# jmhb0/view_neti

Hardware: AMD Instinct MI355X
Metric: TI train steps/sec (SD-1.5 512^2 bs=4 per GPU) (higher is better)
Workload: dtype f16; 1 GPU; learnable_mode 0, sd15 shapes, 512x512 fp16, bs=4/GPU, grad_accum 1, full train step (VAE+16xCLIP+UNet fwd/bwd+AdamW); global_batch=4, parallelism=dp1, rccl_ranks=1, hipgraph=True

## Files before the change

### include/vneti.h

```cpp
#ifndef VNETI_H
#define VNETI_H
#include <stddef.h>
#include <stdint.h>

#ifdef __cplusplus
extern "C" {
#endif

#define VNETI_ABI_VERSION 1

int vneti_version(void);
int vneti_precision(void);
int vneti_last_error(char* buf, size_t n);

typedef struct vneti_gemm_desc {
  const void* A;
  const void* B;
  void* C;
  long long lda, ldb, ldc;
  int M, N, K;
  int batch;
  long long strideA, strideB, strideC;
  const float* bias;
  const void* rowadd;
// ... 65 lines not shown
int vneti_groupnorm_bwd(const void* dy, long long lddy, const void* x, long long ldx,
                        const float* gamma, const float* beta, const float* mean,
                        const float* rstd, void* dx, long long lddx, const void* dx_accum,
                        long long ldacc, float* ws, int Bn, int HW, int C, int G, int silu,
                        void* stream);

int vneti_layernorm_fwd(const void* x, int x_is_f32, long long ldx, void* y, long long ldy,
                        const float* gamma, const float* beta, float* mean, float* rstd, int rows,
                        int C, float eps, void* stream);
int vneti_layernorm_bwd(const void* dy, int dy_is_f32, long long lddy, const void* x,
                        int x_is_f32, long long ldx, const float* gamma, const float* mean,
                        const float* rstd, void* dx, int dx_is_f32, long long lddx,
                        const void* dx_accum, long long ldacc, void* dx_f16_copy, long long ldcopy,
                        int rows, int C, void* stream);

int vneti_attn_fwd(const void* Q, long long ldq, const void* K, long long ldk, const void* V,
                   long long ldv, void* O, long long ldo, float* lse, int Bn, int H, int Nq,
                   int Nk, int D, float scale, int causal, void* stream);
int vneti_attn_bwd_delta(const void* dO, long long lddo, const void* O, long long ldo,
                         float* delta, int Bn, int H, int Nq, int D, void* stream);
int vneti_attn_bwd_dq(const void* Q, long long ldq, const void* K, long long ldk, const void* V,
                      long long ldv, const void* dO, long long lddo, const float* lse, float* delta,
                      const void* O, long long ldo, void* dQ, long long lddq, int Bn, int H, int Nq,
                      int Nk, int D, float scale, int causal, void* stream);
int vneti_attn_bwd_dkv(const void* Q, long long ldq, const void* K, long long ldk, const void* V,
                       long long ldv, const void* dO, long long lddo, const float* lse,
                       const float* delta, void* dK, long long lddk, void* dV, long long lddv,
                       int Bn, int H, int Nq, int Nk, int D, float scale, int causal, float* ws,
                       long long ws_floats, void* stream);
int vneti_attn_bwd_small(const void* Q, long long ldq, const void* K, long long ldk, const void* V, long long ldv,
                         const void* dO, long long lddo, const void* O, long long ldo, const float* lse, void* dQ,
                         long long lddq, void* dK, long long lddk, void* dV, long long lddv, int Bn, int H, int N, int D,
                         float scale, int causal, void* stream);
int vneti_softmax_rows_f16(void* x, long long ld, int rows, int cols, void* stream);

int vneti_add_f16(const void* a, long long lda, const void* b, long long ldb, void* out,
                  long long ldo, int rows, int cols, void* stream);
int vneti_geglu_fwd(const void* p, long long ldp, void* out, long long ldo, int rows, int C4,
                    void* stream);
int vneti_geglu_bwd(const void* dy, long long lddy, const void* p, long long ldp, void* dp,
                    long long lddp, int rows, int C4, void* stream);
int vneti_act_fwd_f16(const void* x, void* y, long long n, int act, void* stream);
int vneti_act_bwd_f16(const void* dy, const void* x, void* dx, long long n, int act, void* stream);
int vneti_timestep_embedding(const void* t, void* out, int Bn, int dim, void* stream);
int vneti_sum2x2_f16(const void* in, long long ldi, void* out, long long ldo, int Bn, int H, int W,
                     int C, void* stream);
int vneti_rng_fill_normal(void* out_f32, long long n, const void* state, unsigned stream_id,
                          void* stream);
int vneti_rng_fill_randint(void* out_i64, int n, int high, const void* state, unsigned stream_id,
                           void* stream);
int vneti_rng_advance(void* state, void* stream);
int vneti_nested_dropout_mask(float* mask, int nl, int Bn, int hidden, float prob, const void* state,
                              unsigned stream_id, void* stream);
int vneti_sample_add_noise(const void* moments, long long ldm, const float* eps,
                           const float* noise, const void* timesteps_i64,
                           const float* alphas_cumprod, float scaling, int v_prediction,
                           float* latents, float* noisy, float* target, int Bn, int Lc, int HW,
                           void* stream);
int vneti_latent_sample(const void* moments, long long ldm, const float* eps, float scaling, float* latents, int Bn,
                        int Lc, int HW, void* stream);
int vneti_add_noise(const float* latents, const float* noise, const void* timesteps_i64, const float* alphas_cumprod,
                    int v_prediction, float* noisy, float* target, int Bn, int Lc, int HW, void* stream);
int vneti_cfg_sampler_step(const void* pred, long long ldp, float* x, float* m_prev, float* x_in, int Bn,
                           int Lc, int HW, float guidance, float alpha_t, float sigma_t, float cx,
                           float c0, float c1, int v_prediction, void* stream);
int vneti_cfg_sampler_step_table(const void* pred, long long ldp, float* x, float* m_prev, float* x_in,
// ... 135 lines not shown
```

### view_neti_amd/csrc/attention.hip

```cpp
#include "common.h"
#include "../../include/vneti.h"

namespace {

constexpr float LOG2E = 1.4426950408889634f;
constexpr int TROW64 = 144;
constexpr int TROW32 = 80;
constexpr int DKV_QH(int D) { return D <= 64 ? 2 : 1; }

template <int D>
struct Cfg {
  static constexpr int KS = (D + 15) / 16;
  static constexpr int DPAD = KS * 16;
  static constexpr int DB = (D + 31) / 32;
  static constexpr int DCH = D / 8;
  static constexpr int ROW = DPAD * 2 + 16;
};

struct AttnArgs {
  const half_t *Q, *K, *V, *dO;
  half_t *O, *dQ, *dK, *dV;
  float* lse;
  const float* lse_in;
  const float* delta;
  float* delta_out;
  const half_t* O_in;
  long long ldq, ldk, ldv, ldo, lddo, lddq, lddk, lddv;
  int Bn, H, Nq, Nk, D;
  float scale;
  int causal;
  int qsplit;
  float* ws;
};

__device__ __forceinline__ float fast_exp2(float x) { return __builtin_amdgcn_exp2f(x); }
typedef float f32x2 __attribute__((ext_vector_type(2)));
__device__ __forceinline__ f32x2 pk_fma(f32x2 a, f32x2 b, f32x2 c) { return __builtin_elementwise_fma(a, b, c); }

constexpr float RESCALE_THR_LOG2 = 8.0f * 1.4426950408889634f;

__device__ __forceinline__ void zero_lds(char* smem, int bytes) {
  u32x4 z = {0u, 0u, 0u, 0u};
  for (int i = threadIdx.x * 16; i < bytes; i += 256 * 16) *reinterpret_cast<u32x4*>(smem + i) = z;
}

__device__ __forceinline__ half8 cvt8(const f32x16& v, int j) {
  half8 h;
#pragma unroll
  for (int e = 0; e < 8; ++e) h[e] = (half_t)v[8 * j + e];
  return h;
}

typedef short vn_short4 __attribute__((__vector_size__(4 * sizeof(short))));
__device__ __forceinline__ half8 load_tr(const char* tile, int row_bytes, int d0, int n0, int lane) {
  const int i = lane & 15;
  const char* p = tile + (n0 + (i >> 2)) * row_bytes + (d0 + 16 * ((lane >> 4) & 1) + 4 * (i & 3)) * 2;
  typedef __attribute__((address_space(3))) vn_short4* lds_ptr;
  vn_short4 lo = __builtin_amdgcn_ds_read_tr16_b64_v4i16((lds_ptr)(p));
  vn_short4 hi = __builtin_amdgcn_ds_read_tr16_b64_v4i16((lds_ptr)(p + 8 * row_bytes));
  half4 l4 = __builtin_bit_cast(half4, lo), h4 = __builtin_bit_cast(half4, hi);
  half8 r = {l4[0], l4[1], l4[2], l4[3], h4[0], h4[1], h4[2], h4[3]};
  return r;
}

template <int D, int QW>
// ... 797 lines not shown
      for (int j = 0; j < 2; ++j) {
        half8 pf = cvt8(s, j);
        half8 dsf = cvt8(dp, j);
#pragma unroll
        for (int db = 0; db < C::DB; ++db) {
          half8 dot = load_tr(dOs, C::ROW, db * 32, hq * 32 + 16 * j + 4 * h2, lane);
          half8 qtf = load_tr(Qs, C::ROW, db * 32, hq * 32 + 16 * j + 4 * h2, lane);
          dv[db] = VN_MFMA_32x32x16(dot, pf, dv[db], 0, 0, 0);
          dk[db] = VN_MFMA_32x32x16(qtf, dsf, dk[db], 0, 0, 0);
        }
      }
    }
    if (rok) {
      half_t* krow = a.dK + ((long long)b * N + row) * a.lddk + h * D;
      half_t* vrow = a.dV + ((long long)b * N + row) * a.lddv + h * D;
#pragma unroll
      for (int db = 0; db < C::DB; ++db)
#pragma unroll
        for (int qd = 0; qd < 4; ++qd) {
          const int d = db * 32 + 8 * qd + 4 * h2;
          if (d < D) {
            half4 k4 = {(half_t)(dk[db][4 * qd] * a.scale), (half_t)(dk[db][4 * qd + 1] * a.scale),
                        (half_t)(dk[db][4 * qd + 2] * a.scale), (half_t)(dk[db][4 * qd + 3] * a.scale)};
            half4 v4 = {(half_t)dv[db][4 * qd], (half_t)dv[db][4 * qd + 1], (half_t)dv[db][4 * qd + 2],
                        (half_t)dv[db][4 * qd + 3]};
            *reinterpret_cast<half4*>(krow + d) = k4;
            *reinterpret_cast<half4*>(vrow + d) = v4;
          }
        }
    }
  }
}

__global__ __launch_bounds__(256) void attn_dkv_reduce_kernel(AttnArgs a) {
  const int Cc = a.H * a.D;
  const long long rows = (long long)a.Bn * a.Nk;
  const long long plane = rows * Cc;
  const unsigned gid = blockIdx.x * 256u + threadIdx.x;
  if (gid >= (unsigned)(plane / 4)) return;
  const unsigned e32 = gid * 4u;
  const unsigned row32 = e32 / (unsigned)Cc;
  const int c = (int)(e32 - row32 * (unsigned)Cc);
  const long long e = e32, row = row32;
  f32x4 k = {0.f, 0.f, 0.f, 0.f}, v = {0.f, 0.f, 0.f, 0.f};
  for (int s = 0; s < a.qsplit; ++s) {
    k += *reinterpret_cast<const f32x4*>(a.ws + ((long long)s * 2) * plane + e);
    v += *reinterpret_cast<const f32x4*>(a.ws + ((long long)s * 2 + 1) * plane + e);
  }
  half4 k4 = {(half_t)(k[0] * a.scale), (half_t)(k[1] * a.scale), (half_t)(k[2] * a.scale), (half_t)(k[3] * a.scale)};
  half4 v4 = {(half_t)v[0], (half_t)v[1], (half_t)v[2], (half_t)v[3]};
  *reinterpret_cast<half4*>(a.dK + row * a.lddk + c) = k4;
  *reinterpret_cast<half4*>(a.dV + row * a.lddv + c) = v4;
}

int check_common(int Bn, int H, int Nq, int Nk, int D) {
  if (Bn <= 0 || H <= 0 || Nq <= 0 || Nk <= 0) return -1;
  if (!(D == 40 || D == 64 || D == 80 || D == 160)) return -2;
  return 0;
}

#define DISPATCH_D(KERNEL, grid, st, args)                                                   \
  switch (args.D) {                                                                          \
    case 40: hipLaunchKernelGGL((KERNEL<40>), grid, dim3(256), 0, st, args); break;          \
    case 64: hipLaunchKernelGGL((KERNEL<64>), grid, dim3(256), 0, st, args); break;          \
    case 80: hipLaunchKernelGGL((KERNEL<80>), grid, dim3(256), 0, st, args); break;          \
    default: hipLaunchKernelGGL((KERNEL<160>), grid, dim3(256), 0, st, args); break;         \
  }

#define DISPATCH_D1(KERNEL, grid, st, args)                                                     \
  switch (args.D) {                                                                             \
    case 40: hipLaunchKernelGGL((KERNEL<40, 1>), grid, dim3(256), 0, st, args); break;          \
    case 64: hipLaunchKernelGGL((KERNEL<64, 1>), grid, dim3(256), 0, st, args); break;          \
    case 80: hipLaunchKernelGGL((KERNEL<80, 1>), grid, dim3(256), 0, st, args); break;          \
    default: hipLaunchKernelGGL((KERNEL<160, 1>), grid, dim3(256), 0, st, args); break;         \
  }

}

extern "C" int vneti_attn_fwd(const void* Q, long long ldq, const void* K, long long ldk, const void* V,
                              long long ldv, void* O, long long ldo, float* lse, int Bn, int H, int Nq, int Nk,
                              int D, float scale, int causal, void* stream) {
  int rc = check_common(Bn, H, Nq, Nk, D);
  VN_REQUIRE(rc == 0, "attn_fwd: unsupported shape B=%d H=%d Nq=%d Nk=%d D=%d", Bn, H, Nq, Nk, D);
  VN_REQUIRE(Q && K && V && O, "attn_fwd: null pointer");
  VN_REQUIRE(ldq % 8 == 0 && ldk % 8 == 0 && ldv % 8 == 0 && ldo % 4 == 0, "attn_fwd: bad strides");
  AttnArgs a;
  memset(&a, 0, sizeof(a));
  a.Q = (const half_t*)Q;
  a.K = (const half_t*)K;
  a.V = (const half_t*)V;
  a.O = (half_t*)O;
  a.lse = lse;
  a.ldq = ldq;
  a.ldk = ldk;
// ... 65 lines not shown
extern "C" int vneti_attn_bwd_dkv(const void* Q, long long ldq, const void* K, long long ldk, const void* V,
                                  long long ldv, const void* dO, long long lddo, const float* lse, const float* delta,
                                  void* dK, long long lddk, void* dV, long long lddv, int Bn, int H, int Nq,
                                  int Nk, int D, float scale, int causal, float* ws, long long ws_floats,
                                  void* stream) {
  int rc = check_common(Bn, H, Nq, Nk, D);
  VN_REQUIRE(rc == 0, "attn_bwd_dkv: unsupported shape B=%d H=%d Nq=%d Nk=%d D=%d", Bn, H, Nq, Nk, D);
  VN_REQUIRE(Q && K && V && dO && lse && delta && dK && dV, "attn_bwd_dkv: null pointer");
  VN_REQUIRE(ldq % 8 == 0 && ldk % 8 == 0 && ldv % 8 == 0 && lddo % 8 == 0 && lddk % 4 == 0 && lddv % 4 == 0,
             "attn_bwd_dkv: bad strides");
  AttnArgs a;
  memset(&a, 0, sizeof(a));
  a.Q = (const half_t*)Q;
  a.K = (const half_t*)K;
  a.V = (const half_t*)V;
  a.dO = (const half_t*)dO;
  a.dK = (half_t*)dK;
  a.dV = (half_t*)dV;
  a.lse_in = lse;
  a.delta = delta;
  a.ldq = ldq;
  a.ldk = ldk;
  a.ldv = ldv;
  a.lddo = lddo;
  a.lddk = lddk;
  a.lddv = lddv;
  a.Bn = Bn;
  a.H = H;
  a.Nq = Nq;
  a.Nk = Nk;
  a.D = D;
  a.scale = scale;
  a.causal = causal;
  const int nkb = cdiv(Nk, 128), nqt = cdiv(Nq, 32 * DKV_QH(D));
  long long blocks = (long long)nkb * H * Bn;
  int qsplit = 1;
  if (ws && !causal && blocks <= 256 && nqt >= 8) {
    qsplit = (int)(512 / blocks);
    if (qsplit > nqt / 4) qsplit = nqt / 4;
    if (qsplit > 32) qsplit = 32;
    const long long plane = (long long)Bn * Nk * H * D;
    while (qsplit > 1 && (2LL * qsplit * plane > ws_floats || 8LL * qsplit * plane >= (1LL << 32) - 64)) --qsplit;
    if (qsplit < 2) qsplit = 1;
  }
  a.qsplit = qsplit;
  a.ws = ws;
  dim3 grid(nkb * qsplit, H, Bn);
  hipStream_t st = (hipStream_t)stream;
  DISPATCH_D(attn_dkv_kernel, grid, st, a);
  if (qsplit > 1) {
    long long n4 = (long long)Bn * Nk * H * D / 4;
    VN_REQUIRE(n4 * 4 < 0x7fffffffLL, "attn_bwd_dkv: q-split reduce indexes with 32 bits");
    hipLaunchKernelGGL(attn_dkv_reduce_kernel, dim3((unsigned)cdivl(n4, 256)), dim3(256), 0, st, a);
  }
  return vneti_check_launch("attn_bwd_dkv");
}

extern "C" int vneti_attn_bwd_small(const void* Q, long long ldq, const void* K, long long ldk, const void* V, long long ldv,
                                    const void* dO, long long lddo, const void* O, long long ldo, const float* lse, void* dQ,
                                    long long lddq, void* dK, long long lddk, void* dV, long long lddv, int Bn, int H, int N,
                                    int D, float scale, int causal, void* stream) {
  VN_REQUIRE(Q && K && V && dO && O && lse && dQ && dK && dV, "attn_bwd_small: null pointer");
  VN_REQUIRE(Bn > 0 && H > 0 && N > 0, "attn_bwd_small: bad shape B=%d H=%d N=%d", Bn, H, N);
  if (N > 96 || D != 64) return VNETI_EUNSUP;
  VN_REQUIRE(ldq % 8 == 0 && ldk % 8 == 0 && ldv % 8 == 0 && lddo % 8 == 0 && ldo % 8 == 0 && lddq % 4 == 0 && lddk % 4 == 0 &&
                 lddv % 4 == 0, "attn_bwd_small: bad strides");
  AttnArgs a;
  memset(&a, 0, sizeof(a));
  a.Q = (const half_t*)Q;
  a.K = (const half_t*)K;
  a.V = (const half_t*)V;
  a.dO = (const half_t*)dO;
  a.O_in = (const half_t*)O;
  a.lse_in = lse;
  a.dQ = (half_t*)dQ;
  a.dK = (half_t*)dK;
  a.dV = (half_t*)dV;
  a.ldq = ldq;
  a.ldk = ldk;
  a.ldv = ldv;
  a.lddo = lddo;
  a.ldo = ldo;
  a.lddq = lddq;
  a.lddk = lddk;
  a.lddv = lddv;
  a.Bn = Bn;
  a.H = H;
  a.Nq = N;
// ... 8 lines not shown
```

### view_neti_amd/engine/schedule.py

```python
from __future__ import annotations

from functools import partial
from typing import Dict, List

import torch

from .. import lib, ops, packing


class T:

    __slots__ = ("v", "g", "gw", "rows", "cols", "children", "need_grad", "producer")

    def __init__(self, v, g=None, need_grad=True):
        self.v = v
        self.g = g
        self.gw = False
        self.rows, self.cols = v.shape
        self.children: List["T"] = []
        self.need_grad = need_grad
        self.producer = None


def rup(x, m):
# ... 135 lines not shown
        conv = f.keywords.get("conv")
        B_cm = packing._chunk_major(f.args[1], f.args[1].shape[0], conv["Ci"]) if _chunk_major_ok(conv) else None
        best, best_t = (0, 0, 0), float("inf")
        for h, sk, ko in gemm_variants(key, conv, f.keywords.get("geglu"), candidates):
            kw = dict(f.keywords)
            kw["tile_hint"], kw["split_k"] = h, sk
            args = f.args
            if ko:
                kw["conv"] = dict(conv, korder=1)
                args = (f.args[0], B_cm) + tuple(f.args[2:])
            t = _time_call(partial(ops.gemm, *args, **kw), args[0], *how)
            if t < best_t:
                best, best_t = (h, sk, ko), t
        return best, B_cm

    def _pin(self, f, pick, B_cm=None):
        pick = tuple(pick) + (0,) * (3 - len(pick))
        conv = f.keywords.get("conv")
        kw = dict(f.keywords)
        kw["tile_hint"], kw["split_k"] = pick[0], pick[1]
        args = f.args
        if pick[2] and _chunk_major_ok(conv):
            if B_cm is None:
                B_cm = packing._chunk_major(f.args[1], f.args[1].shape[0], conv["Ci"])
            kw["conv"] = dict(conv, korder=1)
            self.bytes += B_cm.numel() * B_cm.element_size()
            args = (f.args[0], B_cm) + tuple(f.args[2:])
        return partial(ops.gemm, *args, **kw)

    def bind_workspace(self):
        for lst in (self.fwd_pre, self.fwd, self.bwd):
            for idx, f in enumerate(lst):
                fn = getattr(f, "func", None)
                if fn is ops.gemm or fn is ops.attn_bwd_dkv:
                    lst[idx] = self._rebound(f, fn, dict(f.keywords, workspace=self.ws))

    @staticmethod
    def _rebound(f, fn, kw):
        return partial(fn, *f.args, **kw)

    GN_SLOTS = 8

    def _produced(self, t: T):
        t.producer = len(self.fwd) - 1
        return t

    GN2_MAX = 512

    def _gn2_slice(self):
        if not hasattr(self, "_gn2_arena"):
            self._gn2_arena = self._buf((self.GN2_MAX, self.B, self.GN_SLOTS, self.groups, 4), torch.int64, zero=True)
            self._gn2_used = 0
        assert self._gn2_used < self.GN2_MAX
        self._gn2_used += 1
        return self._gn2_arena[self._gn2_used - 1]

    def fuse_gn_stats(self, fuse: bool = True):
        n = self._fuse_gn_stats() if fuse else 0
        if getattr(self, "_gn2_used", 0):
            self.fwd.insert(0, self._gn2_arena[:self._gn2_used].zero_)
        return n

    def _fuse_gn_stats(self):
        import os
        if os.environ.get("VNETI_NO_GN_FUSE"):
            return 0
        S, G, B = self.GN_SLOTS, self.groups, self.B
# ... 263 lines not shown
```

### view_neti_amd/engine/unet.py

```python
from __future__ import annotations

from functools import partial
from typing import Dict

import torch

from .. import ops, packing
from .. import sd_config as sc
from .schedule import Schedule, T, rup as _rup


class UNetEngine(Schedule):
    def __init__(self, cfg: sc.UNetConfig, weights: Dict[str, torch.Tensor], batch: int, height: int, width: int,
                 ctx_len: int = 77, device: str = "cuda", need_backward: bool = True, autotune: bool = True,
                 fuse_gn: bool = True):
        super().__init__(batch, cfg.norm_num_groups, cfg.norm_eps, device, need_backward)
        self.cfg = cfg
        self.H, self.W = height, width
        self.L = ctx_len
        self.nl = cfg.n_cross_layers
        B, L, Dc = batch, ctx_len, cfg.cross_attention_dim
        self.x_in = self._buf((B, cfg.in_channels, height, width), torch.float32)
        self.timesteps = torch.zeros(B, dtype=torch.int64, device=device)
        self.ctx_k = self._buf((self.nl, B * L, Dc))
# ... 154 lines not shown
            run["wkd"][slot].copy_(w[t + "attn2.to_k.weight"].t())
            run["wvd"][slot].copy_(w[t + "attn2.to_v.weight"].t())
            r["w_outd"] = tr(w[name + "proj_out.weight"].reshape(Cc, Cc))
            r["wff2d"], r["wff1d"] = tr(w[t + "ff.net.2.weight"]), tr(wff1_il)
            r["wo2d"] = tr(w[t + "attn2.to_out.0.weight"])
            if need_dx:
                r["wq2d"] = tr(w[t + "attn2.to_q.weight"])
                r["wo1d"] = tr(w[t + "attn1.to_out.0.weight"])
                r["wqkvd"] = tr(wqkv)
                r["w_ind"] = tr(w_in)
        self.tape.append(r)
        return out

    def _transformer_bwd(self, r):
        B, L, Cc, heads, D, N = self.B, self.L, r["C"], r["heads"], r["D"], r["N"]
        x, out = r["x"], r["out"]
        M = x.rows
        dout = out.g
        assert out.gw, f"transformer {r['name']}: output gradient was never produced"
        li = r["layer"]
        bw = self.bwd
        dh3 = self._tmp("tA", M, Cc)
        bw.append(partial(ops.gemm, dout, r["w_outd"], dh3))
        dp = self._tmp("tC", M, 8 * Cc)
        bw.append(partial(ops.gemm, dh3, r["wff2d"], dp, gate=r["p"], gate_act=ops.ACT_GELU, geglu=2, split_k=1))
        dn3 = self._tmp("tD", M, Cc)
        bw.append(partial(ops.gemm, dp, r["wff1d"], dn3))
        dh2 = self._tmp("tE", M, Cc)
        bw.append(partial(self._ln_bwd, r["ln3"], dn3, dh2, dh3))
        do2 = self._tmp("tA", M, Cc)
        bw.append(partial(ops.gemm, dh2, r["wo2d"], do2))
        delta = self._tmp("tdelta", B * heads, N, torch.float32)
        dq2 = self._tmp("tD", M, Cc)
        if r["need_dx"]:
            bw.append(partial(ops.attn_bwd_dq, r["q2"], r["k2"], r["v2"], do2, r["lse2"], delta, dq2, B, heads, N, L, D,
                              r["scale"], False, O=r["o2"]))
        else:
            bw.append(partial(ops.attn_bwd_delta, do2, r["o2"], delta, B, heads, N, D))
        run, slot = self.kv_slot[li]
        dk2, dv2 = run["dk"][slot], run["dv"][slot]
        bw.append(partial(ops.attn_bwd_dkv, r["q2"], r["k2"], r["v2"], do2, r["lse2"], delta, dk2, dv2, B, heads, N, L,
                          D, r["scale"], False))
        if not r["need_dx"]:
            return
        dn2 = self._tmp("tA", M, Cc)
        bw.append(partial(ops.gemm, dq2, r["wq2d"], dn2))
        dh1 = self._tmp("tF", M, Cc)
        bw.append(partial(self._ln_bwd, r["ln2"], dn2, dh1, dh2))
        do1 = self._tmp("tA", M, Cc)
        bw.append(partial(ops.gemm, dh1, r["wo1d"], do1))
        qkv = r["qkv"]
        q, k, v = qkv[:, :Cc], qkv[:, Cc:2 * Cc], qkv[:, 2 * Cc:]
        dqkv = self._tmp("tC", M, 3 * Cc)
        dq, dk, dv = dqkv[:, :Cc], dqkv[:, Cc:2 * Cc], dqkv[:, 2 * Cc:]
        bw.append(partial(ops.attn_bwd_dq, q, k, v, do1, r["lse1"], delta, dq, B, heads, N, N, D, r["scale"], False,
                          O=r["o1"]))
        bw.append(partial(ops.attn_bwd_dkv, q, k, v, do1, r["lse1"], delta, dk, dv, B, heads, N, N, D, r["scale"],
                          False))
        dn1 = self._tmp("tD", M, Cc)
        bw.append(partial(ops.gemm, dqkv, r["wqkvd"], dn1))
        dh0 = self._tmp("tE", M, Cc)
        bw.append(partial(self._ln_bwd, r["ln1"], dn1, dh0, dh1))
        dg = self._tmp("tA", M, Cc)
        bw.append(partial(ops.gemm, dh0, r["w_ind"], dg))
        self._contrib(x, self._gn_bwd_fn(r["gn"], dg), extra=dout)

    def _upsample(self, x: T, Cc, name, w, out_view, h, wd):
        M = x.rows * 4
        wf = self._w16(packing.conv3x3_fwd(w[name + "weight"]))
        b = self._w32(w[name + "bias"])
        out = T(out_view if out_view is not None else self._buf((M, Cc)))
        self.fwd.append(partial(ops.gemm, x.v, wf, out.v, bias=b, M=M,
                                conv=self._conv_desc(h, wd, Cc, 2 * h, 2 * wd, 1, 1, 1, x.v.stride(0))))
        self._produced(out)
        rec = dict(kind="up", x=x, out=out, C=Cc, h=h, wd=wd)
# ... 155 lines not shown
```

### view_neti_amd/ops.py

```python
from __future__ import annotations

import ctypes as C

import torch

from . import lib as _l

ACT_NONE, ACT_SILU, ACT_QUICK_GELU, ACT_GELU = 0, 1, 2, 3


def stream() -> int:
    return torch.cuda.current_stream().cuda_stream


def _p(t):
    return None if t is None else t.data_ptr()


def _ld(t):
    if t is None:
        return 0
    assert t.stride(-1) == 1, "last dim must be contiguous"
    return t.stride(-2) if t.dim() >= 2 else t.shape[-1]

# ... 131 lines not shown


def attn_fwd(Q, K, V, O, lse, Bn, H, Nq, Nk, D, scale, causal):
    _l.call("attn_fwd", _p(Q), _ld(Q), _p(K), _ld(K), _p(V), _ld(V), _p(O), _ld(O), _p(lse), Bn, H, Nq, Nk, D,
            scale, 1 if causal else 0, stream())


def attn_bwd_delta(dO, O, delta, Bn, H, Nq, D):
    _l.call("attn_bwd_delta", _p(dO), _ld(dO), _p(O), _ld(O), _p(delta), Bn, H, Nq, D, stream())


def attn_bwd_dq(Q, K, V, dO, lse, delta, dQ, Bn, H, Nq, Nk, D, scale, causal, O=None):
    _l.call("attn_bwd_dq", _p(Q), _ld(Q), _p(K), _ld(K), _p(V), _ld(V), _p(dO), _ld(dO), _p(lse), _p(delta),
            _p(O), _ld(O) if O is not None else 0, _p(dQ), _ld(dQ), Bn, H, Nq, Nk, D, scale, 1 if causal else 0,
            stream())


def attn_bwd_dkv(Q, K, V, dO, lse, delta, dK, dV, Bn, H, Nq, Nk, D, scale, causal, workspace=None):
    ws = workspace if workspace is not None else _default_ws
    _l.call("attn_bwd_dkv", _p(Q), _ld(Q), _p(K), _ld(K), _p(V), _ld(V), _p(dO), _ld(dO), _p(lse), _p(delta),
            _p(dK), _ld(dK), _p(dV), _ld(dV), Bn, H, Nq, Nk, D, scale, 1 if causal else 0, _p(ws),
            ws.numel() if ws is not None else 0, stream())


def attn_bwd_small_ok(N, D):
    return N <= 96 and D == 64


def attn_bwd_small(Q, K, V, dO, O, lse, dQ, dK, dV, Bn, H, N, D, scale, causal):
    _l.call("attn_bwd_small", _p(Q), _ld(Q), _p(K), _ld(K), _p(V), _ld(V), _p(dO), _ld(dO), _p(O), _ld(O), _p(lse),
            _p(dQ), _ld(dQ), _p(dK), _ld(dK), _p(dV), _ld(dV), Bn, H, N, D, scale, 1 if causal else 0, stream())


def softmax_rows(x, rows, cols):
    _l.call("softmax_rows_f16", _p(x), _ld(x), rows, cols, stream())


def add(a, b, out):
    rows, cols = out.shape
    _l.call("add_f16", _p(a), _ld(a), _p(b), _ld(b), _p(out), _ld(out), rows, cols, stream())


def geglu_fwd(p, out):
    rows, c4 = out.shape
    _l.call("geglu_fwd", _p(p), _ld(p), _p(out), _ld(out), rows, c4, stream())


def geglu_bwd(dy, p, dp):
    rows, c4 = dy.shape
    _l.call("geglu_bwd", _p(dy), _ld(dy), _p(p), _ld(p), _p(dp), _ld(dp), rows, c4, stream())


def act_fwd(x, y, act):
    _l.call("act_fwd_f16", _p(x), _p(y), x.numel(), act, stream())


def act_bwd(dy, x, dx, act):
    _l.call("act_bwd_f16", _p(dy), _p(x), _p(dx), x.numel(), act, stream())


def timestep_embedding(t, out):
    Bn, dim = out.shape
    _l.call("timestep_embedding", _p(t), _p(out), Bn, dim, stream())


def sum2x2(inp, out, Bn, H, W, Cc):
# ... 330 lines not shown
```

### view_neti_amd/roofline.py

```python
from __future__ import annotations

import torch

from . import ops

import os as _os

_CSRC = _os.path.join(_os.path.dirname(_os.path.abspath(__file__)), "csrc")
MFMA_PEAK_TFLOPS = 2500.0
HBM_PEAK_TBS = 8.0
PF, TB = MFMA_PEAK_TFLOPS, HBM_PEAK_TBS


def kernel_tree_sha() -> str:
    import hashlib
    import os
    here = _CSRC
    files = sorted(os.path.join(here, f) for f in os.listdir(here) if f.endswith((".hip", ".h")))
    files.append(os.path.join(os.path.dirname(os.path.dirname(here)), "include", "vneti.h"))
    h = hashlib.sha256()
    for f in files:
        h.update(os.path.basename(f).encode())
        h.update(open(f, "rb").read())
    return h.hexdigest()[:16]
# ... 7 lines not shown
    batch = kw.get("batch") or 1
    conv = kw.get("conv")
    a_bytes = (M // (conv["Ho"] * conv["Wo"])) * conv["Hi"] * conv["Wi"] * conv["Ci"] * 2 if conv else M * K * 2 * batch
    out = f.args[2]
    c_cols = N * (2 if kw.get("geglu") == 2 else 1)
    extra = sum(M * c * 2 for c, key in ((N, "resid"), (N, "out2"), (c_cols, "gate")) if kw.get(key) is not None)
    if kw.get("geglu") == 1:
        extra -= M * N
    nbytes = a_bytes + N * K * 2 * batch + M * c_cols * out.element_size() * batch + extra
    flops = 2.0 * M * N * K * batch
    return M, N, K, batch, flops, nbytes, flops / (MFMA_PEAK_TFLOPS * 1e12), nbytes / (HBM_PEAK_TBS * 1e12)



def cost(f):
    fn, a, kw = getattr(f, "func", None), getattr(f, "args", ()), getattr(f, "keywords", {}) or {}
    if fn is ops.gemm:
        M, N, K, batch, flops, nbytes, t_mfma, t_hbm = gemm_cost(f)
        if t_hbm > t_mfma:
            return ("gemm, below the ridge (short-K linears: HBM-bound)", 0, nbytes)
        return ("gemm / implicit-GEMM conv (MFMA-bound)", flops, 0)
    if fn in (ops.attn_fwd, ops.attn_bwd_dq, ops.attn_bwd_dkv):
        i = {ops.attn_fwd: 5, ops.attn_bwd_dq: 7, ops.attn_bwd_dkv: 8}[fn]
        Bn, H, Nq, Nk, D = a[i:i + 5]
        causal = a[i + 6]
        mm = {ops.attn_fwd: 2, ops.attn_bwd_dq: 3, ops.attn_bwd_dkv: 4}[fn]
        name = {ops.attn_fwd: "attention fwd", ops.attn_bwd_dq: "attention bwd dQ", ops.attn_bwd_dkv: "attention bwd dK/dV"}[fn]
        scores = Bn * H * Nq * Nk * (0.5 if causal else 1.0)
        ks, db = -(-D // 16), -(-D // 32)
        mfma_c = {ops.attn_fwd: ks + 2 * db, ops.attn_bwd_dq: 2 * ks + 2 * db, ops.attn_bwd_dkv: 2 * ks + 4 * db}[fn] * 32 / 1024.0
        valu_c = {ops.attn_fwd: 2.8, ops.attn_bwd_dq: 4.0, ops.attn_bwd_dkv: 4.0}[fn] * 2 / 64.0 + (2 * 5 / 3) / 64.0
        cob = scores * (mfma_c + valu_c) / (1024 * 2.4e9)
        return (name, mm * 2.0 * scores * D, 0, cob)
    if fn is ops.attn_bwd_small:
        Bn, H, N, D = a[9:13]
        return ("attention bwd (short sequences, one launch)", 7 * 2.0 * Bn * H * N * N * D * (0.5 if a[14] else 1.0), 0)
    if fn in (ops.groupnorm_fwd, ops.groupnorm_fwd_sums, ops.groupnorm_fwd_2l):
        Bn, HW, C = (a[7], a[8], a[9]) if fn is ops.groupnorm_fwd else (a[8], a[9], a[10])
        return ("GroupNorm(+SiLU) fwd" + (" (stats in producer)" if fn is ops.groupnorm_fwd_sums else ""), 0, 2.0 * Bn * HW * C * 2)
    if fn is ops.layernorm_fwd:
        x, y = a[0], a[1]
        return ("LayerNorm fwd", 0, x.numel() * x.element_size() + y.numel() * y.element_size())
    if getattr(f, "vn_cost", None) is not None:
        return (f.vn_cost[0], 0, f.vn_cost[1])
    if getattr(fn, "__name__", "") == "_ln_bwd":
        x = a[0]["x"]
        n = x.numel()
        extra = (a[3].numel() * a[3].element_size() if a[3] is not None else 0) + (n * 2 if len(a) > 4 and a[4] is not None else 0)
        return ("LayerNorm bwd", 0, n * x.element_size() + a[1].numel() * a[1].element_size() + a[2].numel() * a[2].element_size() + extra)
    if fn in (ops.groupnorm_bwd, ops.groupnorm_bwd_2l):
        x = a[1]
        return ("GroupNorm(+SiLU) bwd", 0, 5.0 * x.numel() * 2)
    if fn is ops.add:
        return ("elementwise glue (add, 2x2 sum, transposes, noise, loss)", 0, sum(t.numel() * t.element_size() for t in a[:3]))
    if fn is ops.sum2x2:
        return ("elementwise glue (add, 2x2 sum, transposes, noise, loss)", 0, a[0].numel() * 2 + a[1].numel() * 2)
    if fn in (ops.sample_add_noise, ops.mse_loss_grad, getattr(ops, "transpose", None), getattr(ops, "timestep_embedding", None)):
        return ("elementwise glue (add, 2x2 sum, transposes, noise, loss)", 0,
                sum(t.numel() * t.element_size() for t in a if isinstance(t, torch.Tensor)))
    if fn is ops.layernorm_bwd:
        return ("LayerNorm bwd", 0, sum(t.numel() * t.element_size() for t in (a[0], a[1], a[5])))
    if fn is ops.conv3x3_in:
        return ("VAE conv_in (direct)", 0, a[0].numel() * 4 + a[3].numel() * 2)
    if fn is ops.softmax_rows:
        return ("softmax rows (VAE mid attention)", 0, 2.0 * a[0].numel() * 2)
    if fn is ops.geglu_fwd:
# ... 59 lines not shown
```

Baseline: 39.60 steps/s.

## Fuse cross-attention backward dQ, delta and dK/dV into one kernel

Adds a single-launch backward kernel for cross-attention with short key length (Nk<=96, D 40/80). Each block keeps all keys and values resident and streams query tiles through a double-buffered LDS pipeline. Per tile it computes delta, P, dS, the dK/dV accumulation and dQ, replacing the separate dq/delta and dkv launches. This removes one launch per layer and avoids recomputing the scores twice. It also drops the delta round trip through memory. In exchange it adds LDS pressure and uses only q-split parallelism in the grid.

```diff
diff --git a/include/vneti.h b/include/vneti.h
--- a/include/vneti.h
+++ b/include/vneti.h
@@ -121,6 +121,10 @@
                          const void* dO, long long lddo, const void* O, long long ldo, const float* lse, void* dQ,
                          long long lddq, void* dK, long long lddk, void* dV, long long lddv, int Bn, int H, int N, int D,
                          float scale, int causal, void* stream);
+int vneti_attn_bwd_cross(const void* Q, long long ldq, const void* K, long long ldk, const void* V, long long ldv,
+                         const void* dO, long long lddo, const float* lse, const void* O, long long ldo, void* dQ,
+                         long long lddq, void* dK, long long lddk, void* dV, long long lddv, int Bn, int H, int Nq, int Nk,
+                         int D, float scale, float* ws, long long ws_bytes, int need_dq, void* stream);
 int vneti_softmax_rows_f16(void* x, long long ld, int rows, int cols, void* stream);
 
 int vneti_add_f16(const void* a, long long lda, const void* b, long long ldb, void* out,
diff --git a/view_neti_amd/csrc/attention.hip b/view_neti_amd/csrc/attention.hip
--- a/view_neti_amd/csrc/attention.hip
+++ b/view_neti_amd/csrc/attention.hip
@@ -31,6 +31,7 @@
   int causal;
   int qsplit;
   float* ws;
+  int need_dq;
 };
 
 __device__ __forceinline__ float fast_exp2(float x) { return __builtin_amdgcn_exp2f(x); }
@@ -894,6 +895,277 @@
   }
 }
 
+template <int D>
+__global__ __launch_bounds__(256, 2) void attn_bwd_cross_kernel(AttnArgs a) {
+  using C = Cfg<D>;
+  constexpr int NKR = 96;
+  constexpr int QH = DKV_QH(D), QR = 32 * QH;
+  constexpr int QS_BYTES = QR * C::ROW + 128;
+  constexpr int STAGE = 3 * QS_BYTES + 4 * QR;
+  constexpr int KT_BYTES = NKR * C::ROW + 128;
+  constexpr int DSROW = QH == 2 ? TROW64 : TROW32;
+  constexpr int DS_BYTES = NKR * DSROW;
+  constexpr int SMEM = 2 * STAGE + KT_BYTES + DS_BYTES + 4 * 32 * 4;
+  static_assert(SMEM % 16 == 0 && STAGE % 16 == 0 && KT_BYTES % 16 == 0 && DS_BYTES % 16 == 0, "16-byte LDS accesses");
+  __shared__ __attribute__((aligned(16))) char smem[SMEM];
+  char* Ks = smem + 2 * STAGE;
+  char* dSs = Ks + KT_BYTES;
+  float* dlw = reinterpret_cast<float*>(dSs + DS_BYTES) + 32 * (threadIdx.x >> 6);
+
+  const int tid = threadIdx.x, lane = tid & 63, wave = tid >> 6;
+  const int l31 = lane & 31, h2 = lane >> 5;
+  const int b = blockIdx.z, h = blockIdx.y, qs = blockIdx.x;
+  const int key = wave * 32 + l31;
+  const bool kok = key < a.Nk;
+  const bool kwave = wave * 32 < a.Nk;
+
+  __amdgpu_buffer_rsrc_t rsQ = vn_make_rsrc(a.Q, (uint32_t)((long long)a.Bn * a.Nq * a.ldq * 2));
+  __amdgpu_buffer_rsrc_t rsdO = vn_make_rsrc(a.dO, (uint32_t)((long long)a.Bn * a.Nq * a.lddo * 2));
+  __amdgpu_buffer_rsrc_t rsO = vn_make_rsrc(a.O_in, (uint32_t)((long long)a.Bn * a.Nq * a.ldo * 2));
+  __amdgpu_buffer_rsrc_t rsK = vn_make_rsrc(a.K, (uint32_t)((long long)a.Bn * a.Nk * a.ldk * 2));
+  __amdgpu_buffer_rsrc_t rsV = vn_make_rsrc(a.V, (uint32_t)((long long)a.Bn * a.Nk * a.ldv * 2));
+
+  constexpr int KIT = (NKR * C::DCH + 255) / 256;
+  u32x4 kreg[KIT];
+#pragma unroll
+  for (int i = 0; i < KIT; ++i) {
+    const int idx = tid + 256 * i;
+    const int r = idx / C::DCH, cc = idx - r * C::DCH;
+    const bool ok = idx < NKR * C::DCH && r < a.Nk;
+    kreg[i] = vn_buf_load16(rsK, ok ? (uint32_t)((((long long)b * a.Nk + r) * a.ldk + h * D + cc * 8) * 2) : VN_OOB);
+  }
+  half8 kf[C::KS], vf[C::KS];
+#pragma unroll
+  for (int ks = 0; ks < C::KS; ++ks) {
+    const int ch = ks * 2 + h2;
+    const bool ok = kok && ch < C::DCH;
+    vf[ks] = as_half8(vn_buf_load16(rsV, ok ? (uint32_t)((((long long)b * a.Nk + key) * a.ldv + h * D + ch * 8) * 2) : VN_OOB));
+  }
+  const float c = a.scale * LOG2E;
+
+  constexpr int QIT = (QR * C::DCH + 255) / 256;
+  u32x4 qreg[QIT], doreg[QIT], oreg[QIT];
+  float lreg = INFINITY;
+
+  auto issue = [&](int qt) {
+    const int q0 = qt * QR;
+#pragma unroll
+    for (int i = 0; i < QIT; ++i) {
+      int idx = tid + 256 * i;
+      int r = idx / C::DCH, cc = idx - r * C::DCH;
+      int qq = q0 + r;
+      bool ok = idx < QR * C::DCH && qq < a.Nq;
+      uint32_t o1 = ok ? (uint32_t)((((long long)b * a.Nq + qq) * a.ldq + h * D + cc * 8) * 2) : VN_OOB;
+      uint32_t o2 = ok ? (uint32_t)((((long long)b * a.Nq + qq) * a.lddo + h * D + cc * 8) * 2) : VN_OOB;
+      uint32_t o3 = ok ? (uint32_t)((((long long)b * a.Nq + qq) * a.ldo + h * D + cc * 8) * 2) : VN_OOB;
+      qreg[i] = vn_buf_load16(rsQ, o1);
+      doreg[i] = vn_buf_load16(rsdO, o2);
+      oreg[i] = vn_buf_load16(rsO, o3);
+    }
+    if (tid < QR) {
+      int qq = q0 + tid;
+      lreg = qq < a.Nq ? a.lse_in[((long long)b * a.H + h) * a.Nq + qq] * LOG2E : INFINITY;
+    }
+  };
+  auto commit = [&](int buf) {
+    char* Qs = smem + buf * STAGE;
+    char* dOs = Qs + QS_BYTES;
+    char* Os = dOs + QS_BYTES;
+    float* lses = reinterpret_cast<float*>(Os + QS_BYTES);
+#pragma unroll
+    for (int i = 0; i < QIT; ++i) {
+      int idx = tid + 256 * i;
+      int r = idx / C::DCH, cc = idx - r * C::DCH;
+      if (idx < QR * C::DCH) {
+        *reinterpret_cast<u32x4*>(Qs + r * C::ROW + cc * 16) = qreg[i];
+        *reinterpret_cast<u32x4*>(dOs + r * C::ROW + cc * 16) = doreg[i];
+        *reinterpret_cast<u32x4*>(Os + r * C::ROW + cc * 16) = oreg[i];
+      }
+    }
+    if (tid < QR) lses[tid] = lreg;
+  };
+
+  const int nqt_all = cdiv_dev(a.Nq, QR);
+  const int per = cdiv_dev(nqt_all, a.qsplit);
+  const int nqt = min(nqt_all, (qs + 1) * per);
+  const int qt0 = qs * per;
+  const int nk16 = cdiv_dev(a.Nk, 16);
+
+  if (qt0 < nqt) issue(qt0);
+  zero_lds(smem, SMEM);
+  __syncthreads();
+#pragma unroll
+  for (int i = 0; i < KIT; ++i) {
+    const int idx = tid + 256 * i;
+    const int r = idx / C::DCH, cc = idx - r * C::DCH;
+    if (idx < NKR * C::DCH) *reinterpret_cast<u32x4*>(Ks + r * C::ROW + cc * 16) = kreg[i];
+  }
+  if (qt0 < nqt) commit(0);
+  __syncthreads();
+  f32x16 dk[C::DB], dv[C::DB];
+#pragma unroll
+  for (int i = 0; i < C::DB; ++i)
+#pragma unroll
+    for (int e = 0; e < 16; ++e) {
+      dk[i][e] = 0.f;
+      dv[i][e] = 0.f;
+    }
+
+#pragma unroll
+  for (int ks = 0; ks < C::KS; ++ks)
+    kf[ks] = as_half8(*reinterpret_cast<const u32x4*>(Ks + (kwave ? key : 0) * C::ROW + (ks * 2 + h2) * 16));
+
+  for (int qt = qt0; qt < nqt; ++qt) {
+    if (qt + 1 < nqt) issue(qt + 1);
+    const int q0 = qt * QR;
+    const char* Qs = smem + ((qt - qt0) & 1) * STAGE;
+    const char* dOs = Qs + QS_BYTES;
+    const char* Os = dOs + QS_BYTES;
+    const float* lses = reinterpret_cast<const float*>(Os + QS_BYTES);
+
+    if (kwave) {
+#pragma unroll
+      for (int hq = 0; hq < QH; ++hq) {
+        f32x16 s, dp;
+#pragma unroll
+        for (int e = 0; e < 16; ++e) {
+          s[e] = 0.f;
+          dp[e] = 0.f;
+        }
+        float part = 0.f;
+#pragma unroll
+        for (int ks = 0; ks < C::KS; ++ks) {
+          const int off = (hq * 32 + l31) * C::ROW + (ks * 2 + h2) * 16;
+          half8 qfr = as_half8(*reinterpret_cast<const u32x4*>(Qs + off));
+          half8 dofr = as_half8(*reinterpret_cast<const u32x4*>(dOs + off));
+          s = VN_MFMA_32x32x16(qfr, kf[ks], s, 0, 0, 0);
+          dp = VN_MFMA_32x32x16(dofr, vf[ks], dp, 0, 0, 0);
+          if (a.need_dq) {
+            half8 of = as_half8(*reinterpret_cast<const u32x4*>(Os + off));
+#pragma unroll
+            for (int j = 0; j < 8; ++j) part += (float)dofr[j] * (float)of[j];
+          }
+        }
+        if (a.need_dq) {
+          part = part + __shfl_xor(part, 32, 64);
+        } else {
+          const char* po = Os + (hq * 32 + l31) * C::ROW;
+          const char* pd = dOs + (hq * 32 + l31) * C::ROW;
+          for (int cc = 0; cc < C::DCH; ++cc) {
+            half8 x = as_half8(*reinterpret_cast<const u32x4*>(po + cc * 16));
+            half8 y = as_half8(*reinterpret_cast<const u32x4*>(pd + cc * 16));
+#pragma unroll
+            for (int j = 0; j < 8; ++j) part += (float)x[j] * (float)y[j];
+          }
+        }
+        dlw[l31] = part;
+#pragma unroll
+        for (int qd = 0; qd < 4; ++qd) {
+          f32x4 l4 = *reinterpret_cast<const f32x4*>(&lses[hq * 32 + 8 * qd + 4 * h2]);
+          f32x4 d4 = *reinterpret_cast<const f32x4*>(&dlw[8 * qd + 4 * h2]);
+#pragma unroll
+          for (int e = 0; e < 4; e += 2) {
+            const int r = 4 * qd + e;
+            const f32x2 t = pk_fma(f32x2{s[r], s[r + 1]}, f32x2{c, c}, -f32x2{l4[e], l4[e + 1]});
+            const f32x2 p = f32x2{fast_exp2(t.x), fast_exp2(t.y)};
+            const f32x2 ds = p * (f32x2{dp[r], dp[r + 1]} - f32x2{d4[e], d4[e + 1]});
+            s[r] = p.x;
+            s[r + 1] = p.y;
+            dp[r] = ds.x;
+            dp[r + 1] = ds.y;
+          }
+        }
+#pragma unroll
+        for (int j = 0; j < 2; ++j) {
+          half8 pf = cvt8(s, j);
+          half8 dsf = cvt8(dp, j);
+#pragma unroll
+          for (int db = 0; db < C::DB; ++db) {
+            half8 dot = load_tr(dOs, C::ROW, db * 32, hq * 32 + 16 * j + 4 * h2, lane);
+            half8 qtf = load_tr(Qs, C::ROW, db * 32, hq * 32 + 16 * j + 4 * h2, lane);
+            dv[db] = VN_MFMA_32x32x16(dot, pf, dv[db], 0, 0, 0);
+            dk[db] = VN_MFMA_32x32x16(qtf, dsf, dk[db], 0, 0, 0);
+          }
+          if (a.need_dq) {
+#pragma unroll
+            for (int u = 0; u < 2; ++u) {
+              half4 d4h = {dsf[4 * u], dsf[4 * u + 1], dsf[4 * u + 2], dsf[4 * u + 3]};
+              if (!kok) d4h = half4{(half_t)0.f, (half_t)0.f, (half_t)0.f, (half_t)0.f};
+              *reinterpret_cast<half4*>(dSs + key * DSROW + (hq * 32 + 8 * (2 * j + u) + 4 * h2) * 2) = d4h;
+            }
+          }
+        }
+      }
+    }
+    if (a.need_dq) {
+      __syncthreads();
+      for (int p = wave; p < QH * C::DB; p += 4) {
+        const int qb = p / C::DB, db = p - qb * C::DB;
+        f32x16 dq;
+#pragma unroll
+        for (int e = 0; e < 16; ++e) dq[e] = 0.f;
+        for (int kk = 0; kk < nk16; ++kk) {
+          half8 tf = load_tr(Ks, C::ROW, db * 32, kk * 16 + 4 * h2, lane);
+          half8 pf = load_tr(dSs, DSROW, qb * 32, kk * 16 + 4 * h2, lane);
+          dq = VN_MFMA_32x32x16(tf, pf, dq, 0, 0, 0);
+        }
+        const int q = q0 + qb * 32 + l31;
+        if (q < a.Nq) {
+          half_t* orow = a.dQ + ((long long)b * a.Nq + q) * a.lddq + h * D;
+#pragma unroll
+          for (int qd = 0; qd < 4; ++qd) {
+            const int d = db * 32 + 8 * qd + 4 * h2;
+            if (d < D) {
+              half4 v = {(half_t)(dq[4 * qd] * a.scale), (half_t)(dq[4 * qd + 1] * a.scale),
+                         (half_t)(dq[4 * qd + 2] * a.scale), (half_t)(dq[4 * qd + 3] * a.scale)};
+              *reinterpret_cast<half4*>(orow + d) = v;
+            }
+          }
+        }
+      }
+    }
+    if (qt + 1 < nqt) commit((qt + 1 - qt0) & 1);
+    __syncthreads();
+  }
+
+  if (!kok) return;
+  if (a.qsplit > 1) {
+    const long long plane = (long long)a.Bn * a.Nk * a.H * D;
+    const __amdgpu_buffer_rsrc_t rsP = vn_make_rsrc(a.ws, 0xfffffff0u);
+#pragma unroll
+    for (int db = 0; db < C::DB; ++db)
+#pragma unroll
+      for (int qd = 0; qd < 4; ++qd) {
+        int d = db * 32 + 8 * qd + 4 * h2;
+        if (d < D) {
+          f32x4 k4 = {dk[db][4 * qd], dk[db][4 * qd + 1], dk[db][4 * qd + 2], dk[db][4 * qd + 3]};
+          f32x4 v4 = {dv[db][4 * qd], dv[db][4 * qd + 1], dv[db][4 * qd + 2], dv[db][4 * qd + 3]};
+          const uint32_t po = (uint32_t)(((((long long)qs * 2) * plane + ((long long)b * a.Nk + key) * (a.H * D) + h * D + d)) * 4);
+          vn_st16_wt(rsP, po, k4);
+          vn_st16_wt(rsP, po + (uint32_t)(plane * 4), v4);
+        }
+      }
+    return;
+  }
+  half_t* krow = a.dK + ((long long)b * a.Nk + key) * a.lddk + h * D;
+  half_t* vrow = a.dV + ((long long)b * a.Nk + key) * a.lddv + h * D;
+#pragma unroll
+  for (int db = 0; db < C::DB; ++db) {
+#pragma unroll
+    for (int qd = 0; qd < 4; ++qd) {
+      int d = db * 32 + 8 * qd + 4 * h2;
+      if (d < D) {
+        half4 k4 = {(half_t)(dk[db][4 * qd] * a.scale), (half_t)(dk[db][4 * qd + 1] * a.scale),
+                    (half_t)(dk[db][4 * qd + 2] * a.scale), (half_t)(dk[db][4 * qd + 3] * a.scale)};
+        half4 v4 = {(half_t)dv[db][4 * qd], (half_t)dv[db][4 * qd + 1], (half_t)dv[db][4 * qd + 2],
+                    (half_t)dv[db][4 * qd + 3]};
+        *reinterpret_cast<half4*>(krow + d) = k4;
+        *reinterpret_cast<half4*>(vrow + d) = v4;
+      }
+    }
+  }
+}
+
 __global__ __launch_bounds__(256) void attn_dkv_reduce_kernel(AttnArgs a) {
   const int Cc = a.H * a.D;
   const long long rows = (long long)a.Bn * a.Nk;
@@ -921,7 +1193,22 @@
   return 0;
 }
 
-#define DISPATCH_D(KERNEL, grid, st, args)                                                   \
+int dkv_qsplit(int Bn, int H, int Nq, int Nk, int D, int causal, const float* ws, long long ws_floats) {
+  const int nkb = cdiv(Nk, 128), nqt = cdiv(Nq, 32 * DKV_QH(D));
+  long long blocks = (long long)nkb * H * Bn;
+  int qsplit = 1;
+  if (ws && !causal && blocks <= 256 && nqt >= 8) {
+    qsplit = (int)(512 / blocks);
+    if (qsplit > nqt / 4) qsplit = nqt / 4;
+    if (qsplit > 32) qsplit = 32;
+    const long long plane = (long long)Bn * Nk * H * D;
+    while (qsplit > 1 && (2LL * qsplit * plane > ws_floats || 8LL * qsplit * plane >= (1LL << 32) - 64)) --qsplit;
+    if (qsplit < 2) qsplit = 1;
+  }
+  return qsplit;
+}
+
+#define DISPATCH_D(KERNEL, grid, st, args)                                                  \
   switch (args.D) {                                                                          \
     case 40: hipLaunchKernelGGL((KERNEL<40>), grid, dim3(256), 0, st, args); break;          \
     case 64: hipLaunchKernelGGL((KERNEL<64>), grid, dim3(256), 0, st, args); break;          \
@@ -1053,17 +1340,8 @@
   a.D = D;
   a.scale = scale;
   a.causal = causal;
-  const int nkb = cdiv(Nk, 128), nqt = cdiv(Nq, 32 * DKV_QH(D));
-  long long blocks = (long long)nkb * H * Bn;
-  int qsplit = 1;
-  if (ws && !causal && blocks <= 256 && nqt >= 8) {
-    qsplit = (int)(512 / blocks);
-    if (qsplit > nqt / 4) qsplit = nqt / 4;
-    if (qsplit > 32) qsplit = 32;
-    const long long plane = (long long)Bn * Nk * H * D;
-    while (qsplit > 1 && (2LL * qsplit * plane > ws_floats || 8LL * qsplit * plane >= (1LL << 32) - 64)) --qsplit;
-    if (qsplit < 2) qsplit = 1;
-  }
+  const int nkb = cdiv(Nk, 128);
+  const int qsplit = dkv_qsplit(Bn, H, Nq, Nk, D, causal, ws, ws_floats);
   a.qsplit = qsplit;
   a.ws = ws;
   dim3 grid(nkb * qsplit, H, Bn);
@@ -1075,6 +1353,63 @@
     hipLaunchKernelGGL(attn_dkv_reduce_kernel, dim3((unsigned)cdivl(n4, 256)), dim3(256), 0, st, a);
   }
   return vneti_check_launch("attn_bwd_dkv");
+}
+
+extern "C" int vneti_attn_bwd_cross(const void* Q, long long ldq, const void* K, long long ldk, const void* V,
+                                    long long ldv, const void* dO, long long lddo, const float* lse, const void* O,
+                                    long long ldo, void* dQ, long long lddq, void* dK, long long lddk, void* dV,
+                                    long long lddv, int Bn, int H, int Nq, int Nk, int D, float scale, float* ws,
+                                    long long ws_bytes, int need_dq, void* stream) {
+  VN_REQUIRE(Bn > 0 && H > 0 && Nq > 0 && Nk > 0, "attn_bwd_cross: bad shape B=%d H=%d Nq=%d Nk=%d", Bn, H, Nq, Nk);
+  if (Nk > 96 || !(D == 40 || D == 80)) {
+    vneti_set_error("attn_bwd_cross: unsupported shape Nk=%d D=%d (Nk <= 96, D = 40 or 80)", Nk, D);
+    return VNETI_EUNSUP;
+  }
+  VN_REQUIRE(Q && K && V && dO && lse && O && dK && dV && (dQ || !need_dq), "attn_bwd_cross: null pointer");
+  VN_REQUIRE(ldq % 8 == 0 && ldk % 8 == 0 && ldv % 8 == 0 && lddo % 8 == 0 && ldo % 8 == 0 && lddq % 4 == 0 &&
+                 lddk % 4 == 0 && lddv % 4 == 0, "attn_bwd_cross: bad strides");
+  VN_REQUIRE(ws_bytes >= 0 && (ws || ws_bytes == 0), "attn_bwd_cross: ws_bytes without ws");
+  AttnArgs a;
+  memset(&a, 0, sizeof(a));
+  a.Q = (const half_t*)Q;
+  a.K = (const half_t*)K;
+  a.V = (const half_t*)V;
+  a.dO = (const half_t*)dO;
+  a.O_in = (const half_t*)O;
+  a.lse_in = lse;
+  a.dQ = (half_t*)dQ;
+  a.dK = (half_t*)dK;
+  a.dV = (half_t*)dV;
+  a.ldq = ldq;
+  a.ldk = ldk;
+  a.ldv = ldv;
+  a.lddo = lddo;
+  a.ldo = ldo;
+  a.lddq = lddq;
+  a.lddk = lddk;
+  a.lddv = lddv;
+  a.Bn = Bn;
+  a.H = H;
+  a.Nq = Nq;
+  a.Nk = Nk;
+  a.D = D;
+  a.scale = scale;
+  a.need_dq = need_dq ? 1 : 0;
+  const int qsplit = dkv_qsplit(Bn, H, Nq, Nk, D, 0, ws, ws_bytes / 4);
+  a.qsplit = qsplit;
+  a.ws = ws;
+  dim3 grid(qsplit, H, Bn);
+  hipStream_t st = (hipStream_t)stream;
+  if (qsplit > 1) VN_REQUIRE((long long)Bn * Nk * H * D < 0x7fffffffLL, "attn_bwd_cross: q-split reduce indexes with 32 bits");
+  switch (D) {
+    case 40: hipLaunchKernelGGL((attn_bwd_cross_kernel<40>), grid, dim3(256), 0, st, a); break;
+    default: hipLaunchKernelGGL((attn_bwd_cross_kernel<80>), grid, dim3(256), 0, st, a); break;
+  }
+  if (qsplit > 1) {
+    long long n4 = (long long)Bn * Nk * H * D / 4;
+    hipLaunchKernelGGL(attn_dkv_reduce_kernel, dim3((unsigned)cdivl(n4, 256)), dim3(256), 0, st, a);
+  }
+  return vneti_check_launch("attn_bwd_cross");
 }
 
 extern "C" int vneti_attn_bwd_small(const void* Q, long long ldq, const void* K, long long ldk, const void* V, long long ldv,
diff --git a/view_neti_amd/engine/schedule.py b/view_neti_amd/engine/schedule.py
--- a/view_neti_amd/engine/schedule.py
+++ b/view_neti_amd/engine/schedule.py
@@ -191,7 +191,7 @@
         for lst in (self.fwd_pre, self.fwd, self.bwd):
             for idx, f in enumerate(lst):
                 fn = getattr(f, "func", None)
-                if fn is ops.gemm or fn is ops.attn_bwd_dkv:
+                if fn is ops.gemm or fn is ops.attn_bwd_dkv or fn is ops.attn_bwd_cross:
                     lst[idx] = self._rebound(f, fn, dict(f.keywords, workspace=self.ws))
 
     @staticmethod
diff --git a/view_neti_amd/engine/unet.py b/view_neti_amd/engine/unet.py
--- a/view_neti_amd/engine/unet.py
+++ b/view_neti_amd/engine/unet.py
@@ -210,15 +210,20 @@
         bw.append(partial(ops.gemm, dh2, r["wo2d"], do2))
         delta = self._tmp("tdelta", B * heads, N, torch.float32)
         dq2 = self._tmp("tD", M, Cc)
-        if r["need_dx"]:
-            bw.append(partial(ops.attn_bwd_dq, r["q2"], r["k2"], r["v2"], do2, r["lse2"], delta, dq2, B, heads, N, L, D,
-                              r["scale"], False, O=r["o2"]))
-        else:
-            bw.append(partial(ops.attn_bwd_delta, do2, r["o2"], delta, B, heads, N, D))
         run, slot = self.kv_slot[li]
         dk2, dv2 = run["dk"][slot], run["dv"][slot]
-        bw.append(partial(ops.attn_bwd_dkv, r["q2"], r["k2"], r["v2"], do2, r["lse2"], delta, dk2, dv2, B, heads, N, L,
-                          D, r["scale"], False))
+        if ops.attn_bwd_cross_ok(L, D):
+            bw.append(partial(ops.attn_bwd_cross, r["q2"], r["k2"], r["v2"], do2, r["o2"], r["lse2"],
+                              dq2 if r["need_dx"] else None, dk2, dv2, B, heads, N, L, D, r["scale"],
+                              need_dq=r["need_dx"]))
+        else:
+            if r["need_dx"]:
+                bw.append(partial(ops.attn_bwd_dq, r["q2"], r["k2"], r["v2"], do2, r["lse2"], delta, dq2, B, heads, N, L,
+                                  D, r["scale"], False, O=r["o2"]))
+            else:
+                bw.append(partial(ops.attn_bwd_delta, do2, r["o2"], delta, B, heads, N, D))
+            bw.append(partial(ops.attn_bwd_dkv, r["q2"], r["k2"], r["v2"], do2, r["lse2"], delta, dk2, dv2, B, heads, N,
+                              L, D, r["scale"], False))
         if not r["need_dx"]:
             return
         dn2 = self._tmp("tA", M, Cc)
diff --git a/view_neti_amd/ops.py b/view_neti_amd/ops.py
--- a/view_neti_amd/ops.py
+++ b/view_neti_amd/ops.py
@@ -187,6 +187,17 @@
             _p(dQ), _ld(dQ), _p(dK), _ld(dK), _p(dV), _ld(dV), Bn, H, N, D, scale, 1 if causal else 0, stream())
 
 
+def attn_bwd_cross_ok(Nk, D):
+    return Nk <= 96 and D in (40, 80)
+
+
+def attn_bwd_cross(Q, K, V, dO, O, lse, dQ, dK, dV, Bn, H, Nq, Nk, D, scale, need_dq=True, workspace=None):
+    ws = workspace if workspace is not None else _default_ws
+    _l.call("attn_bwd_cross", _p(Q), _ld(Q), _p(K), _ld(K), _p(V), _ld(V), _p(dO), _ld(dO), _p(lse), _p(O), _ld(O),
+            _p(dQ), _ld(dQ), _p(dK), _ld(dK), _p(dV), _ld(dV), Bn, H, Nq, Nk, D, scale, _p(ws),
+            ws.numel() * ws.element_size() if ws is not None else 0, 1 if need_dq else 0, stream())
+
+
 def softmax_rows(x, rows, cols):
     _l.call("softmax_rows_f16", _p(x), _ld(x), rows, cols, stream())
 
diff --git a/view_neti_amd/roofline.py b/view_neti_amd/roofline.py
--- a/view_neti_amd/roofline.py
+++ b/view_neti_amd/roofline.py
@@ -63,6 +63,15 @@
         valu_c = {ops.attn_fwd: 2.8, ops.attn_bwd_dq: 4.0, ops.attn_bwd_dkv: 4.0}[fn] * 2 / 64.0 + (2 * 5 / 3) / 64.0
         cob = scores * (mfma_c + valu_c) / (1024 * 2.4e9)
         return (name, mm * 2.0 * scores * D, 0, cob)
+    if fn is ops.attn_bwd_cross:
+        Bn, H, Nq, Nk, D = a[9:14]
+        dq = 1 if kw.get("need_dq", True) else 0
+        scores = Bn * H * Nq * Nk
+        ks, db = -(-D // 16), -(-D // 32)
+        mfma_c = (2 * ks + (4 + 2 * dq) * db) * 32 / 1024.0
+        valu_c = 4.0 * 2 / 64.0 + (2 * 5 / 3) / 64.0
+        cob = scores * (mfma_c + valu_c) / (1024 * 2.4e9)
+        return ("attention bwd (cross, one launch)", (4 + dq) * 2.0 * scores * D, 0, cob)
     if fn is ops.attn_bwd_small:
         Bn, H, N, D = a[9:13]
         return ("attention bwd (short sequences, one launch)", 7 * 2.0 * Bn * H * N * N * D * (0.5 if a[14] else 1.0), 0)
```

New measurement: 39.61 steps/s (median of 3 runs). About the same (+0.0%).
